# kuboyoo/alphazero-general-ori

Measured on AMD Instinct MI355X. Metric: self-play rollouts/sec (32k boards, 2p Splendor) at 1/2/4/8 MI355X, higher is better.
Workload: dtype fp32 (network) / int8 (boards) / f64 (tree statistics)

## Files before the change

alphazero-general-ori_amd/csrc/mcts.hip:

```cpp
#include <hip/hip_runtime.h>

#include <cmath>
#include <cstring>
#include <new>

#include "../../include/splendor_amd.h"

#include "board_phases.h"
#include "mcts_device.h"
#include "nn_stage.h"
#include "spl_ctx.h"

using namespace spl;

#ifndef SPL_BOUNDS_CHECK
#define SPL_BOUNDS_CHECK 0
#endif
#if SPL_BOUNDS_CHECK
__device__ unsigned long long g_bounds[4 + 64];
__device__ __noinline__ void bounds_note(int site, long long v, int t) {
    atomicAdd(&g_bounds[4 + (site & 63)], 1ull);
    if (atomicAdd(&g_bounds[0], 1ull) == 0) {
        g_bounds[1] = (unsigned long long)v; g_bounds[2] = (unsigned long long)site; g_bounds[3] = (unsigned long long)t;
    }
// ... 477 lines not shown
            const int cl = c >= 0 ? node_l(P, c) : -1;
            const bool fresh = cl >= 0 && atomicCAS(&mark[cl], 0, 1) == 0;
            const uint64_t bm = __ballot(fresh);
            if (fresh) q[tail + __popcll(bm & lanemask_lt())] = cl;
            tail += __popcll(bm);
            wave_lds_fence();
        }
    }
}

typedef uint32_t u32x4 __attribute__((ext_vector_type(4)));
struct NodeRaw {
    u32x4 q[4];
    __device__ __forceinline__ int bchild() const { return (int)q[0].x; }
    __device__ __forceinline__ bool term() const { return (q[1].y & 0xFFu) != 0; }
    __device__ __forceinline__ uint64_t ebq() const { return (uint64_t)q[2].x | ((uint64_t)q[2].y << 32); }
    __device__ __forceinline__ uint64_t vbq() const { return (uint64_t)q[2].z | ((uint64_t)q[2].w << 32); }
    __device__ __forceinline__ int ec() const { return (int)(int16_t)(q[3].x & 0xFFFFu); }
    __device__ __forceinline__ void set_runs(uint64_t e, uint64_t v) {
        q[2] = u32x4{(uint32_t)e, (uint32_t)(e >> 32), (uint32_t)v, (uint32_t)(v >> 32)};
    }
    __device__ __forceinline__ void clear_hints() { q[0].y = 0xFFFFFFFFu; q[0].z = 0xFFFFFFFFu; }
};
static_assert(sizeof(NodeRaw) == sizeof(Node) && offsetof(Node, h.bchild) == 0 && offsetof(Node, h.h2) == 4 &&
                  offsetof(Node, h.h3) == 8 && offsetof(Node, h.term) == 20 && offsetof(Node, c.ebq) == 32 &&
                  offsetof(Node, c.vbq) == 40 && offsetof(Node, c.ec) == 48,
              "NodeRaw's field offsets");

constexpr int GCT = 512, GCW8 = GCT / 64;
struct GcLds {
    int32_t wsum[GCW8];
    int32_t bc[4];
};
__device__ __forceinline__ int block_scan(int x, int &total, GcLds &L) {
    const int l = lane_id(), w = threadIdx.x >> 6;
    int incl = x;
#pragma unroll
    for (int o = 1; o < 64; o <<= 1) {
        const int y = __shfl_up(incl, o, 64);
        if (l >= o) incl += y;
    }
    if (l == 63) L.wsum[w] = incl;
    __syncthreads();
    int off = 0, tot = 0;
#pragma unroll
    for (int i = 0; i < GCW8; i++) {
// ... 842 lines not shown
        b ^= mix64(x ^ 0x13198A2E03707344ull);
    }
    k0 = a;
    k1 = b | 1ull;
}
template <int N>
__device__ __forceinline__ void lane_tree_step(int8_t *s, int a) {
    Chance ch{nullptr, 0, 0, 0, 0};
    int nxt;
    switch (move_kind_of(a)) {
        case MK_GEMS: nxt = make_move<N, MK_GEMS>(s, a, 0, true, ch); break;
        case MK_BUY: nxt = make_move<N, MK_BUY>(s, a, 0, true, ch); break;
        case MK_RESERVE: nxt = make_move<N, MK_RESERVE>(s, a, 0, true, ch); break;
        default: nxt = make_move<N, MK_BUY_RESERVED>(s, a, 0, true, ch); break;
    }
    if (nxt) lane_roll_players<N>(s, nxt);
}

#ifndef SELECT_PROBE
#define SELECT_PROBE 0
#endif
#if SELECT_PROBE
__device__ unsigned long long g_sel_probe[16];
#define SPROBE(k)                                                  \
    {                                                              \
        const uint64_t c_ = __builtin_readcyclecounter();          \
        pacc[k] += c_ - plast;                                     \
        plast = c_;                                                \
    }
#else
#define SPROBE(k)
#endif
#ifndef PATH_CHUNK
#define PATH_CHUNK 8
#endif
enum { LS_DESCEND = 0, LS_EXPAND = 1, LS_DONE = 2 };

#ifndef SELECT_ASM
#define SELECT_ASM 1
#endif
#define SEL_STORES 2
#define SEL_W_OWN 3
#define SEL_W_HINT 8
#define SEL_W_HINT1 9
static_assert(SEL_W_OWN == 1 + SEL_STORES, "own child load: behind SC + the stores");
static_assert(SEL_W_HINT == SEL_STORES + 2 * (1 + SEL_STORES) && SEL_W_HINT1 == SEL_W_HINT + 1,
              "hinted record: two levels back");
#define SEL_STR2(x) #x
#define SEL_STR(x) SEL_STR2(x)
#define SEL_BODY(SA, SC, K)                                                                     \
    "v_cmp_le_i32 vcc, 0, v240\n"                       \
    "v_cmp_le_i32 %[T], 0, v243\n"                      \
    "s_and_b64 vcc, vcc, %[T]\n"                                                               \
    "v_cmp_gt_i32 %[T], %[pcap], v233\n"                \
    "s_and_b64 vcc, vcc, %[T]\n"                                                               \
    "s_and_b64 exec, exec, vcc\n"                                                              \
    "s_cbranch_execz L_done_%=\n"                                                              \
    "v_cmp_ne_u32 vcc, v240, v234\n"                  \
    "s_and_saveexec_b64 %[SV], vcc\n"                   \
    "s_mov_b64 %[INV], exec\n"                                                                 \
    "s_cbranch_execz L_nf" K "_%=\n"                                                           \
    "v_mad_u64_u32 v[238:239], %[CC], v240, 64, %[nd]\n"                                       \
    "global_load_dwordx4 " SA ", v[238:239], off\n"                                            \
    "L_nf" K "_%=:\n"                                                                          \
    "s_mov_b64 exec, %[SV]\n"                                                                  \
    "v_cmp_gt_u32 vcc, %[lim], v242\n"                  \
    "v_cndmask_b32 v226, v240, v242, vcc\n"             \
    "v_mad_u64_u32 v[238:239], %[CC], v226, 64, %[nd]\n"                                       \
    "global_load_dwordx4 " SC ", v[238:239], off\n"                                            \
    "v_mad_u64_u32 v[238:239], %[CC], v233, 4, v[252:253]\n"         \
    "global_store_dword v[238:239], v232, off\n"                                               \
    "v_and_b32 v236, 0xffff, v243\n"                                \
    "v_bfe_u32 v237, v243, 16, 15\n"                                                           \
    "v_lshl_or_b32 v236, v237, 9, v236\n"                                                      \
    "v_mad_u64_u32 v[238:239], %[CC], v233, 4, v[254:255]\n"                                   \
    "global_store_dword v[238:239], v236, off\n"                                               \
    "v_add_u32 v233, 1, v233\n"                                                                \
    "v_mov_b32 v232, v240\n"                                                                   \
    "v_mov_b32 v234, v235\n"                       \
    "v_mov_b32 v235, v226\n"                                                                   \
    "s_cmp_eq_u64 %[INV], 0\n"                                                                 \
    "s_cbranch_scc1 L_av" K "_%=\n"                                                            \
    "s_waitcnt vmcnt(" SEL_STR(SEL_W_OWN) ")\n"          \
    "s_mov_b32 %[F], 1\n"                                                                      \
    "s_branch L_sel" K "_%=\n"                                                                 \
    "L_av" K "_%=:\n"                                   \
    "s_cmp_eq_u32 %[F], 0\n"                            \
    "s_cbranch_scc1 L_a8" K "_%=\n"                     \
    "s_waitcnt vmcnt(" SEL_STR(SEL_W_HINT1) ")\n"                                              \
    "s_branch L_a0" K "_%=\n"                                                                  \
    "L_a8" K "_%=:\n"                                                                          \
    "s_waitcnt vmcnt(" SEL_STR(SEL_W_HINT) ")\n"                                               \
    "L_a0" K "_%=:\n"                                                                          \
    "s_mov_b32 %[F], 0\n"                                                                      \
    "L_sel" K "_%=:\n"
#define SEL_TAKE(R)                                                                             \
    "v_mov_b32 v240, v" #R "\n"                                                                \
    "v_mov_b32 v241, v" #R "+1\n"
__device__ __forceinline__ void descend_linked_asm(int &node, int &depth, NodeLink &rec, const Node *nd, int pcap,
                                                   int32_t *path_n, int32_t *path_x, uint64_t runm, int lim) {
    int r0 = rec.bchild, r1 = rec.h2, r2 = rec.h3;
    int r3 = (int)((uint32_t)(uint16_t)rec.best | ((uint32_t)rec.babt << 16));
    uint64_t T, SV, INV, CC, SAVE;
    int F;
    asm volatile(
        "s_mov_b64 %[SAVE], exec\n"
        "s_mov_b32 %[F], 1\n"
        "v_mov_b32 v232, %[node]\n"
        "v_mov_b32 v233, %[depth]\n"
        "v_mov_b32 v240, %[r0]\n"
        "v_mov_b32 v241, %[r1]\n"
        "v_mov_b32 v242, %[r2]\n"
        "v_mov_b32 v243, %[r3]\n"
        "v_mov_b32 v234, -1\n"
        "v_mov_b32 v235, -1\n"
        "v_mov_b64 v[252:253], %[pn]\n"
        "v_mov_b64 v[254:255], %[pxp]\n"
        "s_and_b64 exec, exec, %[runm]\n"
        "s_cbranch_execz L_done_%=\n"
        "L_top_%=:\n"
        SEL_BODY("v[244:247]", "v[228:231]", "0")
        "v_mov_b32 v240, v244\n" "v_mov_b32 v241, v245\n" "v_mov_b32 v242, v246\n" "v_mov_b32 v243, v247\n"
        SEL_BODY("v[248:251]", "v[244:247]", "1")
        "v_mov_b32 v240, v248\n" "v_mov_b32 v241, v249\n" "v_mov_b32 v242, v250\n" "v_mov_b32 v243, v251\n"
        SEL_BODY("v[228:231]", "v[248:251]", "2")
        "v_mov_b32 v240, v228\n" "v_mov_b32 v241, v229\n" "v_mov_b32 v242, v230\n" "v_mov_b32 v243, v231\n"
        "s_branch L_top_%=\n"
        "L_done_%=:\n"
        "s_waitcnt vmcnt(0)\n"
        "s_mov_b64 exec, %[SAVE]\n"
        "v_mov_b32 %[node], v232\n"
        "v_mov_b32 %[depth], v233\n"
        "v_mov_b32 %[r0], v240\n"
        "v_mov_b32 %[r1], v241\n"
        "v_mov_b32 %[r2], v242\n"
        "v_mov_b32 %[r3], v243\n"
        : [node] "+v"(node), [depth] "+v"(depth), [r0] "+v"(r0), [r1] "+v"(r1), [r2] "+v"(r2), [r3] "+v"(r3),
          [T] "=&s"(T), [SV] "=&s"(SV), [INV] "=&s"(INV), [CC] "=&s"(CC), [SAVE] "=&s"(SAVE), [F] "=&s"(F)
        : [nd] "s"(nd), [pcap] "s"(pcap), [pn] "v"(path_n), [pxp] "v"(path_x), [runm] "s"(runm), [lim] "s"(lim)
        : "v226", "v227", "v228", "v229", "v230", "v231", "v232", "v233", "v234", "v235", "v236", "v237", "v238",
          "v239", "v240", "v241", "v242", "v243", "v244", "v245", "v246", "v247", "v248", "v249", "v250", "v251",
          "v252", "v253", "v254", "v255", "vcc", "scc", "memory");
    rec.bchild = r0; rec.h2 = r1; rec.h3 = r2;
    rec.best = (int16_t)(r3 & 0xFFFF); rec.babt = (uint16_t)((uint32_t)r3 >> 16);
}
#undef SEL_BODY
#undef SEL_TAKE

template <int N>
__global__ __launch_bounds__(64) void k_select_lanes(Pools P, SearchCfg C, int B, int lim,
                                                     int8_t *__restrict__ leaf_state,
                                                     uint8_t *__restrict__ leaf_valid) {
    using Lx = Lay<N>;
    constexpr int ST = (Lx::ROWS % 2 ? Lx::ROWS : Lx::ROWS + 1) * 8;
    __shared__ __align__(16) int8_t boards[64 * ST];
    __shared__ RunScr scr;
    const int l = lane_id();
#if SELECT_PROBE
    uint64_t pacc[6] = {0, 0, 0, 0, 0, 0}, plast = __builtin_readcyclecounter();
    const uint64_t pstart = plast;
    int plev = 0, pexp = 0;
#endif
    const int slot = blockIdx.x * 64 + l;
    const bool live = slot < B;
    const int t = live ? slot : 0;
    TreeHdr *H = P.hdr + t;
    int8_t *s = boards + l * ST;
    int sims = 0, root = -1, hdepth = 0, mv = 0, hnc = 0, hnpg = 0;
    bool act = false, noise = false, forced = false;
    if (live) {
        sims = H->sims_done;
        act = sims < H->budget && !H->overflow;
        root = H->root; hdepth = H->depth; mv = H->move_no;
        noise = H->noise_pending != 0; forced = H->forced != 0;
        hnc = H->node_count; hnpg = H->npg;
        if (!act) { leaf_valid[t] = 0; H->leaf_kind = LEAF_NONE; }
    }
    const uint64_t *nbrd = reinterpret_cast<const uint64_t *>(P.nbrd);
    const int32_t pstride = P.pcap + 1;
    int32_t *path_n = P.path_n + (size_t)t * pstride;
    int32_t *path_x = P.path_x + (size_t)t * P.pcap;
    if (act && (root < 0 || !nbrd))
        for (int u = 0; u < Conv<N>::UNITS; u++) Conv<N>::load(s, P.root_state + (size_t)t * Lx::S, u);
    const bool noised = act && root >= 0 && sims == 0 && noise;
// ... 35 lines not shown
    for (uint64_t m = __ballot(scan); m; m &= m - 1) {
        const int j = __ffsll((unsigned long long)m) - 1;
        const int nj = __builtin_amdgcn_readlane(node, j);
        NodeRun r = run_of(P.nd[nj].c);
        r.eb = (int64_t)uniform64((uint64_t)r.eb); r.vb = (int64_t)uniform64((uint64_t)r.vb);
        r.ec = uniform(r.ec);
        const Pick p = scan_run(P, r, __builtin_amdgcn_readlane(nsq.ns, j), readlane_f64(nsq.qs, j), C.cpuct, C.fpu,
                                __builtin_amdgcn_readlane((int)forced, j) != 0, __builtin_amdgcn_readlane(sims, j));
        if (l == j) { pk = p; have_pk = true; }
    }
    if (have_pk) {
        if (pk.child < 0 && pk.e == nsq.best && !noised) { pk.child = nsq.bchild; pk.cterm = nsq.bterm(); }
        else pk.cterm = pk.child >= 0 ? (int)P.nd[pk.child].h.term : 0;
    }
    int bnode = nbrd ? -1 : node;
    int miss = -1, leaf_node = -1, cbest = -1;
    uint64_t k0 = 0, k1 = 0;
    float val[4] = {0, 0, 0, 0};
    NodeLink rec = *reinterpret_cast<const NodeLink *>(&nsq);
    int tv_node = -1;
    SPROBE(0)
    while (__ballot(state != LS_DONE)) {
      while (__ballot(state == LS_DESCEND)) {
        bool run = state == LS_DESCEND && !have_pk && nbrd;
#if SELECT_ASM
        {
#if SELECT_PROBE || SPL_BOUNDS_CHECK
            const int d0 = depth;
#endif
            descend_linked_asm(node, depth, rec, P.nd, P.pcap, path_n, path_x, __ballot(run), P.npages * NPG);
#if SELECT_PROBE
            plev += depth - d0;
#endif
#if SPL_BOUNDS_CHECK
            for (int d = d0; d < depth; d++) {
                const int pn = path_n[d], c = d + 1 < depth ? path_n[d + 1] : node;
                BCHK(IN_TREE(P, t, c, H->node_count), 52, c, t, (void)0);
                BCHK(P.nd[c].h.round == P.nd[pn].h.round + 1, 30, ((long long)pn << 32) | (uint32_t)c, t, (void)0);
            }
#endif
            run = false;
        }
#endif
        while (__ballot(run)) {
            if (run) {
                const int c = rec.bchild;
                run = c >= 0 && !rec.bterm() && depth < P.pcap;
                if (run) {
                    BCHK(IN_TREE(P, t, c, H->node_count), 52, c, t, (void)0);
                    BCHK(P.nd[c].h.round == P.nd[node].h.round + 1, 30, ((long long)node << 32) | (uint32_t)c, t, (void)0);
                    const NodeLink nx = link_of(P.nd, c);
                    path_n[depth] = node; path_x[depth] = px_pack(rec.best, rec.ba());
                    depth++;
                    node = c;
                    rec = nx;
#if SELECT_PROBE
                    plev++;
#endif
                }
            }
        }
        if (state == LS_DESCEND) {
            if (depth >= P.pcap) {
                state = LS_DONE; kind = LEAF_NONE; H->overflow = 2;
            } else {
                if (!have_pk) pk = Pick{rec.best, rec.ba(), rec.bchild, rec.bterm()};
                have_pk = false;
                cbest = rec.best;
#if SELECT_PROBE
                plev++;
#endif
                path_n[depth] = node; path_x[depth] = px_pack(pk.e, pk.a);
                depth++;
                if (pk.child >= 0 && pk.cterm) {
                    kind = LEAF_TERMINAL;
                    leaf_node = pk.child;
                    tv_node = pk.child;
                    state = LS_DONE;
                } else if (pk.child >= 0 && nbrd) {
                    BCHK(IN_TREE(P, t, pk.child, H->node_count), 52, pk.child, t, (void)0);
                    rec = link_of(P.nd, pk.child);
                    node = pk.child;
                } else {
// ... 103 lines not shown
#pragma unroll
        for (int i = 0; i < 4; i++) H->leaf_v[i] = val[i];
        leaf_valid[t] = kind == LEAF_NN;
        path_n[depth] = kind == LEAF_TERMINAL ? leaf_node : -1;
    }
#if SELECT_PROBE
    SPROBE(4)
    if (l == 0) {
        for (int k = 0; k < 5; k++) atomicAdd(&g_sel_probe[k], (unsigned long long)pacc[k]);
        atomicAdd(&g_sel_probe[5], 1ull);
        atomicMax(&g_sel_probe[6], (unsigned long long)(plast - pstart));
        atomicAdd(&g_sel_probe[7], (unsigned long long)(plast - pstart));
    }
    {
        const int lmax = wave_max_i32(plev);
        int lsum = plev;
#pragma unroll
        for (int o = 32; o > 0; o >>= 1) lsum += __shfl_xor(lsum, o, 64);
        if (l == 0) {
            atomicAdd(&g_sel_probe[8], (unsigned long long)lmax);
            atomicAdd(&g_sel_probe[9], (unsigned long long)lsum);
            atomicMax(&g_sel_probe[10], (unsigned long long)lmax);
            atomicAdd(&g_sel_probe[11], (unsigned long long)pexp);
        }
    }
#endif
}

#ifndef LM_PROBE
#define LM_PROBE 0
#endif
#if LM_PROBE
constexpr int LM_PSLOTS = 4096;
__device__ unsigned long long g_lm_probe[LM_PSLOTS][8];
#define LMPROBE(k) \
    if (threadIdx.x == 0 && blockIdx.x < LM_PSLOTS) g_lm_probe[blockIdx.x][k] = __builtin_amdgcn_s_memrealtime();
#else
#define LMPROBE(k)
#endif
__device__ __forceinline__ int nonzero_bytes(uint32_t x) {
    return __popc((((x & 0x7F7F7F7Fu) + 0x7F7F7F7Fu) | x) & 0x80808080u);
}
template <int N, bool STG = false>
__global__ __launch_bounds__(256) void k_leaf_mask(Pools P, int B, int lim, const int8_t *__restrict__ leaf_state,
                                                   const uint8_t *__restrict__ leaf_valid,
                                                   uint64_t *__restrict__ leaf_mask,
// ... 971 lines not shown
        }
        if (threadIdx.x < N)
            v[(size_t)t * N + threadIdx.x] =
                (float)((threadIdx.x == 0 ? 1.0 : -1.0) *
                        (1.0 - (double)(mix64(h ^ (0xA5A5ull + threadIdx.x)) >> 40) * 0x1p-30));
        return;
    }
    for (int a = threadIdx.x; a < SPL_ACTIONS; a += 256) {
        const bool ok = (mask[(size_t)t * 7 + a / 64] >> (a % 64)) & 1;
        pi[(size_t)t * SPL_ACTIONS + a] =
            ok ? (float)((double)(1 + (mix64(h + (uint64_t)a) >> 40)) * 0x1p-24) : 0.f;
    }
    if (threadIdx.x < N)
        v[(size_t)t * N + threadIdx.x] =
            (float)((double)(mix64(h ^ (0xA5A5ull + threadIdx.x)) >> 40) * 0x1p-23 - 1.0);
}

__global__ void k_init_pools(Pools P, int B) {
    const size_t tid = (size_t)blockIdx.x * blockDim.x + threadIdx.x, nth = (size_t)gridDim.x * blockDim.x;
    const int nsh = P.npages - P.nhome * B, esh = P.epages - P.ehome * B;
    for (size_t i = tid; i < (size_t)nsh; i += nth) P.nfree[i] = (int32_t)(P.npages - 1 - i);
    for (size_t i = tid; i < (size_t)esh; i += nth) P.efree[i] = (int32_t)(P.epages - 1 - i);
    if (tid == 0) { P.alloc[0] = nsh; P.alloc[1] = esh; P.alloc[2] = 0; P.alloc[3] = 0; }
}

inline int check_launch() { return hipGetLastError() == hipSuccess ? 0 : SPL_EDEVICE; }
inline dim3 wave_grid(int B) { return dim3((unsigned)((B + WAVES - 1) / WAVES)); }

#define SPL_DISPATCH(n, CALL)                          \
    switch (n) {                                       \
        case 2: { constexpr int N = 2; CALL; break; }  \
        case 3: { constexpr int N = 3; CALL; break; }  \
        default: { constexpr int N = 4; CALL; break; } \
    }

template <class T>
T *carve(char *&p, size_t count) {
    T *r = reinterpret_cast<T *>(p);
    size_t bytes = (count * sizeof(T) + 255) & ~size_t(255);
    p += bytes;
    return r;
}

}

extern "C" {
// ... 36 lines not shown
    acc(16 * no); acc(64); acc((size_t)L.nbb * nn); acc(4 * (size_t)B); acc(4 * (size_t)B); acc(8 * no);
    L.bytes = bytes;
    return L;
}

static bool valid_cfg(const spl_ctx *ctx, int B, const spl_mcts_config *cfg) {
    if (!(ok_ctx(ctx) && B > 0 && cfg && cfg->num_sims > 0 && cfg->ratio_full > 0 &&
          cfg->node_cap > 0 && cfg->edge_cap > 0 && cfg->pool_nodes >= 0 && cfg->pool_edges >= 0))
        return false;
    const long long nmax = (long long)((cfg->node_cap + NPG - 1) / NPG) * NPG;
    const long long emax = (long long)((cfg->edge_cap + UPG - 1) / UPG) * UPG;
    const long long pn = cfg->pool_nodes > 0 ? cfg->pool_nodes : (long long)B * nmax;
    const long long pe = cfg->pool_edges > 0 ? cfg->pool_edges : (long long)B * emax;
    return cfg->node_cap <= (1 << 24) && cfg->edge_cap <= (1 << 28) && pn + NPG < (1LL << 31) &&
           pe / UPG + 1 < (1LL << 31);
}

#if SELECT_PROBE
int spl_diag_select_probe(unsigned long long *out16, int reset) {
    if (hipMemcpyFromSymbol(out16, HIP_SYMBOL(g_sel_probe), 16 * 8) != hipSuccess) return SPL_EDEVICE;
    if (reset) {
        unsigned long long z[16] = {0};
        if (hipMemcpyToSymbol(HIP_SYMBOL(g_sel_probe), z, sizeof(z)) != hipSuccess) return SPL_EDEVICE;
    }
    return 0;
}
#endif

#if GC_PROBE
int spl_diag_gc_probe(unsigned long long *out24, int reset) {
    static unsigned long long h[GC_WG_MAX_PROBE][16], hm[GC_WG_MAX_PROBE][8];
    if (hipMemcpyFromSymbol(h, HIP_SYMBOL(g_gc_probe), sizeof(h)) != hipSuccess) return SPL_EDEVICE;
    if (hipMemcpyFromSymbol(hm, HIP_SYMBOL(g_gc_probe_max), sizeof(hm)) != hipSuccess) return SPL_EDEVICE;
    for (int k = 0; k < 24; k++) out24[k] = 0;
    for (int i = 0; i < GC_WG_MAX_PROBE; i++) {
        for (int k = 0; k < 10; k++) out24[k] += h[i][k];
        if (h[i][10] > out24[10]) {
            for (int k = 10; k < 14; k++) out24[k] = h[i][k];
            for (int k = 0; k < 7; k++) out24[16 + k] = hm[i][k];
        }
    }
    if (reset) {
        memset(h, 0, sizeof(h));
        memset(hm, 0, sizeof(hm));
        if (hipMemcpyToSymbol(HIP_SYMBOL(g_gc_probe), h, sizeof(h)) != hipSuccess) return SPL_EDEVICE;
        if (hipMemcpyToSymbol(HIP_SYMBOL(g_gc_probe_max), hm, sizeof(hm)) != hipSuccess) return SPL_EDEVICE;
// ... 148 lines not shown
    const int prev = g_gc_lds_limit;
    g_gc_lds_limit = nodes < 0 ? -1 : nodes;
    return prev;
}

int spl_mcts_set_roots_active(spl_mcts *m, const int8_t *roots, const uint8_t *active, int keep_tree,
                              int force_full, void *hs) {
    if (!m || !roots) return SPL_EINVAL;
    SPL_DISPATCH(m->n, hipLaunchKernelGGL(k_set_roots<N>, wave_grid(m->B), dim3(THREADS), 0,
                                          (hipStream_t)hs, m->P, m->cfg, m->B, roots, active, keep_tree,
                                          force_full));
    launch_gc(m, (hipStream_t)hs);
    return check_launch();
}

int spl_mcts_pick_best(spl_mcts *m, const uint8_t *active, uint32_t board_base, uint32_t stream,
                       int16_t *action, void *hs) {
    if (!m || !action || stream > 0xFFFFFFu) return SPL_EINVAL;
    hipLaunchKernelGGL(k_pick_best, wave_grid(m->B), dim3(THREADS), 0, (hipStream_t)hs, m->P, m->cfg,
                       m->B, active, board_base, stream, action);
    return check_launch();
}

static int launch_select(spl_mcts *m, int8_t *leaf_state, uint64_t *leaf_mask, uint8_t *leaf_valid,
                         int32_t *leaf_index, int32_t *leaf_count, void *hs) {
    SPL_DISPATCH(m->n, hipLaunchKernelGGL(k_select_lanes<N>, dim3((unsigned)((m->B + 63) / 64)), dim3(64), 0,
                                          (hipStream_t)hs, m->P, m->cfg, m->B, mcts_lim(m),
                                          leaf_state, leaf_valid));
    char *no_stage = nullptr;
    SPL_DISPATCH(m->n, hipLaunchKernelGGL(k_leaf_mask<N>, dim3((unsigned)((m->B + 63) / 64)), dim3(256), 0,
                                          (hipStream_t)hs, m->P, m->B, mcts_lim(m), leaf_state, leaf_valid,
                                          leaf_mask, leaf_index, leaf_count, no_stage));
    return check_launch();
}

static int launch_mask_staged(int n, const Pools &P, int B, int lim, const int8_t *leaf_state,
                              const uint8_t *leaf_valid, uint64_t *leaf_mask, void *stage, void *hs) {
    int32_t *no_list = nullptr;
    char *st = static_cast<char *>(stage);
    SPL_DISPATCH(n, hipLaunchKernelGGL((k_leaf_mask<N, true>), dim3((unsigned)((B + 63) / 64)), dim3(256), 0,
                                       (hipStream_t)hs, P, B, lim, leaf_state, leaf_valid, leaf_mask, no_list,
                                       no_list, st));
    return check_launch();
}
static bool stage_args_ok(const void *leaf_state, const void *leaf_mask, const void *leaf_valid, const void *stage) {
    return leaf_state && leaf_mask && leaf_valid && stage && reinterpret_cast<uintptr_t>(leaf_state) % 4 == 0 &&
           reinterpret_cast<uintptr_t>(leaf_mask) % 8 == 0 && reinterpret_cast<uintptr_t>(leaf_valid) % 16 == 0 &&
           reinterpret_cast<uintptr_t>(stage) % 16 == 0;
}

int spl_mcts_select_staged(spl_mcts *m, int8_t *leaf_state, uint64_t *leaf_mask, uint8_t *leaf_valid, void *stage,
                           void *hs) {
    if (!m || !stage_args_ok(leaf_state, leaf_mask, leaf_valid, stage)) return SPL_EINVAL;
    SPL_DISPATCH(m->n, hipLaunchKernelGGL(k_select_lanes<N>, dim3((unsigned)((m->B + 63) / 64)), dim3(64), 0,
                                          (hipStream_t)hs, m->P, m->cfg, m->B, mcts_lim(m),
                                          leaf_state, leaf_valid));
    return launch_mask_staged(m->n, m->P, m->B, mcts_lim(m), leaf_state, leaf_valid, leaf_mask, stage, hs);
}

int spl_nn_stage_leaves(const spl_ctx *ctx, int B, const int8_t *leaf_state, const uint8_t *leaf_valid,
                        uint64_t *leaf_mask, void *stage, void *hs) {
    if (!ok_ctx(ctx) || B < 0 || !stage_args_ok(leaf_state, leaf_mask, leaf_valid, stage))
        return SPL_EINVAL;
    if (!B) return 0;
    return launch_mask_staged(ctx->n, Pools{}, B, pack_lim(ctx->token_limit, ctx->rules), leaf_state, leaf_valid,
                              leaf_mask, stage, hs);
}

int spl_mcts_select(spl_mcts *m, int8_t *leaf_state, uint64_t *leaf_mask, uint8_t *leaf_valid,
                    void *hs) {
    if (!m || !leaf_state || !leaf_mask || !leaf_valid) return SPL_EINVAL;
    return launch_select(m, leaf_state, leaf_mask, leaf_valid, nullptr, nullptr, hs);
}

int spl_mcts_select_compact(spl_mcts *m, int8_t *leaf_state, uint64_t *leaf_mask, uint8_t *leaf_valid,
                            int32_t *leaf_index, int32_t *leaf_count, void *hs) {
    if (!m || !leaf_state || !leaf_mask || !leaf_valid || !leaf_index || !leaf_count) return SPL_EINVAL;
    return launch_select(m, leaf_state, leaf_mask, leaf_valid, leaf_index, leaf_count, hs);
// ... 135 lines not shown
```

alphazero-general-ori_amd/csrc/mcts_device.h:

```cpp
#pragma once
#include "splendor_device.h"

namespace spl {

constexpr double Q_UNSET = -42.0;

struct TreeHdr {
    int32_t node_count, edge_count, root, sims_done;
    int32_t budget, full, noise_pending, depth;
    int32_t leaf_kind, player, episode_step, move_no;
    int32_t game_no, overflow, n_examples, leaf_round;
    uint64_t leaf_k0, leaf_k1;
    float leaf_v[4];
    int32_t games_done, forced, moves, wd_search;
    int32_t prunes, resets, unexpanded, gc_state;
    int64_t units_gc;
    int64_t enext;
    int32_t npg, epg, eleft, live_gc;
    int32_t root_round, gc_queued, withdrawals, gcs;
    int32_t leaf_hslot, leaf_slot;
    int32_t depth_max, depth_sum;
    int32_t resume;
    int32_t sims_backed, exact_wide, big_moves;
};
// ... 149 lines not shown
__device__ __forceinline__ int64_t unit_g(const Pools &P, int t, int v) {
    const int pi = v >> UPG_SHIFT;
    const int64_t pg = pi < P.ehome ? (int64_t)t * P.ehome + pi : (int64_t)P.etab[(size_t)t * P.eptab + pi];
    return pg * UPG + (v & (UPG - 1));
}

template <int N>
struct NodeBoard {
    static constexpr int BYTES = (Lay<N>::LS + 15) & ~15;
    static constexpr int UNITS = BYTES / 16;
};

struct SearchCfg {
    double cpuct, fpu, dir_alpha, dir_temp, prob_full;
    int num_sims, ratio_full, forced_playouts, dirichlet;
    int temp_threshold, selfplay;
    int edge_reserve;
    uint64_t seed;
    uint32_t board_base;
};

enum : uint32_t { ST_FULL = 1u << 24, ST_DIR = 2u << 24, ST_PICK = 3u << 24, ST_MOVE = 4u << 24,
                  ST_DEAL = 5u << 24, ST_BEST = 6u << 24,
                  ST_PLAYER = 8u << 24 };

__device__ __forceinline__ uint64_t wave_xor64(uint64_t x) {
#pragma unroll
    for (int o = 32; o > 0; o >>= 1) x ^= __shfl_xor(x, o, 64);
    return x;
}

__device__ __forceinline__ void wave_argmax(double &u, int &i) {
#pragma unroll
    for (int o = 32; o > 0; o >>= 1) {
        double u2 = __shfl_xor(u, o, 64);
        int i2 = __shfl_xor(i, o, 64);
        if (u2 > u || (u2 == u && i2 < i)) { u = u2; i = i2; }
    }
}

template <int CTRL>
__device__ __forceinline__ double dpp_f64(double v) {
    const int lo = __double2loint(v), hi = __double2hiint(v);
    return __hiloint2double(__builtin_amdgcn_update_dpp(hi, hi, CTRL, 0xF, 0xF, false),
                            __builtin_amdgcn_update_dpp(lo, lo, CTRL, 0xF, 0xF, false));
}
__device__ __forceinline__ double wave_max_f64(double v) {
// ... 202 lines not shown
```

alphazero-general-ori_amd/splendor/_lib.py:

```python
import ctypes as C
import os

PKG_ROOT = os.path.dirname(os.path.dirname(os.path.abspath(__file__)))
LIB_PATH = os.environ.get("SPLENDOR_AMD_LIB") or os.path.join(PKG_ROOT, "libsplendor_amd.so")

ABI_VERSION = 11
EINVAL, EDEVICE = -1, -2
ERR_BAD_ACTION, ERR_BAD_INDEX = 1, 2
BACKUP_DEFER_GC = 4
PLAYER_RANDOM, PLAYER_GREEDY, PLAYER_POLICY = 0, 1, 2
PLAYOUT_UNIFORM, PLAYOUT_BUY_FIRST = 0, 1
RULE_NO_RESERVE = 1


class NativeEngineMissing(RuntimeError):
    pass


class EngineError(RuntimeError):
    pass


_lib = None

# ... 39 lines not shown
                     C.c_uint32, _vp, _vp, _vp, _vp, _vp], C.c_int),
    "spl_playout_seq": ([C.c_void_p, C.c_int, _vp, _vp, _vp, _vp, C.c_int, C.c_int, C.c_int, C.c_uint64, _vp,
                         C.c_uint32, _vp, _vp, _vp, _vp, _vp], C.c_int),
    "spl_playout_mix": ([C.c_void_p, C.c_int, _vp, _vp, _vp, _vp, C.c_int, C.c_int, C.c_int, C.c_uint64, _vp,
                         C.c_uint32, _vp, _vp, _vp, _vp], C.c_int),
    "spl_mcts_create": ([C.c_void_p, C.c_int, C.c_void_p, C.POINTER(C.c_void_p)], C.c_int),
    "spl_mcts_destroy": ([C.c_void_p], C.c_int),
    "spl_mcts_device_bytes": ([C.c_void_p], C.c_longlong),
    "spl_mcts_plan_bytes": ([_vp, C.c_int, _vp], C.c_longlong),
    "spl_mcts_counters": ([C.c_void_p, _vp, _vp], C.c_int),
    "spl_mcts_pool_state": ([C.c_void_p, _vp, _vp], C.c_int),
    "spl_mcts_pool_pages": ([C.c_void_p, _vp], C.c_int),
    "spl_mcts_set_roots": ([C.c_void_p, _vp, C.c_int, C.c_int, _vp], C.c_int),
    "spl_mcts_set_roots_active": ([C.c_void_p, _vp, _vp, C.c_int, C.c_int, _vp], C.c_int),
    "spl_mcts_pick_best": ([C.c_void_p, _vp, C.c_uint32, C.c_uint32, _vp, _vp], C.c_int),
    "spl_mcts_select": ([C.c_void_p, _vp, _vp, _vp, _vp], C.c_int),
    "spl_mcts_select_compact": ([C.c_void_p, _vp, _vp, _vp, _vp, _vp, _vp], C.c_int),
    "spl_mcts_backup": ([C.c_void_p, _vp, _vp, _vp, _vp], C.c_int),
    "spl_mcts_backup_kind": ([C.c_void_p, _vp, _vp, _vp, C.c_int, _vp], C.c_int),
    "spl_mcts_root_stats": ([C.c_void_p, _vp, _vp, _vp, _vp, _vp, _vp], C.c_int),
    "spl_mcts_root_priors": ([C.c_void_p, _vp, _vp], C.c_int),
    "spl_mcts_headers": ([C.c_void_p, _vp, _vp], C.c_int),
    "spl_mcts_tree_sizes": ([C.c_void_p, _vp, _vp], C.c_int),
    "spl_mcts_reset_games": ([C.c_void_p, _vp], C.c_int),
    "spl_mcts_restart_games": ([C.c_void_p, _vp, _vp], C.c_int),
    "spl_mcts_commit": ([C.c_void_p, _vp], C.c_int),
    "spl_mcts_drain_examples": ([C.c_void_p, _vp, _vp, _vp, _vp, _vp, _vp, _vp, C.c_int, _vp, _vp], C.c_int),
    "spl_nn_input": ([C.c_void_p, C.c_int, _vp, _vp, _vp, _vp, _vp], C.c_int),
    "spl_hash_eval": ([C.c_void_p, C.c_int, _vp, _vp, _vp, _vp, _vp], C.c_int),
    "spl_hash_eval_mode": ([C.c_void_p, C.c_int, _vp, _vp, _vp, _vp, C.c_int, _vp], C.c_int),
}


class MctsConfig(C.Structure):
    _fields_ = [("num_sims", C.c_int), ("ratio_full", C.c_int), ("prob_full", C.c_double),
                ("cpuct", C.c_double), ("fpu", C.c_double), ("forced_playouts", C.c_int),
                ("dirichlet_alpha", C.c_double), ("dirichlet_temp", C.c_double),
                ("temp_threshold", C.c_int), ("node_cap", C.c_int), ("edge_cap", C.c_int),
                ("seed", C.c_uint64), ("board_base", C.c_uint32), ("selfplay", C.c_int),
                ("out_cap", C.c_int), ("node_boards", C.c_int), ("pool_nodes", C.c_longlong),
                ("pool_edges", C.c_longlong)]


def exported_symbols():
    return list(_SIGS)

# ... 27 lines not shown
```

include/splendor_amd.h:

```cpp
#ifndef SPLENDOR_AMD_H
#define SPLENDOR_AMD_H
#include <stdint.h>
#ifdef __cplusplus
extern "C" {
#endif

#define SPL_ABI_VERSION 11
#define SPL_ACTIONS 409
#define SPL_MASK_WORDS 7
#define SPL_EINVAL (-1)
#define SPL_EDEVICE (-2)
#define SPL_ERR_BAD_ACTION 1
#define SPL_ERR_BAD_INDEX 2

typedef struct spl_ctx spl_ctx;

int spl_abi_version(void);

int spl_ctx_create(int n_players, int token_limit, spl_ctx **out);
int spl_ctx_destroy(spl_ctx *ctx);
int spl_ctx_set_token_limit(spl_ctx *ctx, int token_limit);
#define SPL_RULE_NO_RESERVE 1
int spl_ctx_set_rules(spl_ctx *ctx, int flags);
int spl_ctx_rules(const spl_ctx *ctx);
// ... 118 lines not shown
int spl_mcts_backup(spl_mcts *m, const uint64_t *leaf_mask, const float *pi, const float *v,
                    void *hip_stream);
#define SPL_LEAF_NN 1
#define SPL_LEAF_TERMINAL 2
#define SPL_BACKUP_DEFER_GC 4
int spl_mcts_backup_kind(spl_mcts *m, const uint64_t *leaf_mask, const float *pi, const float *v, int kinds,
                         void *hip_stream);
int spl_mcts_root_priors(spl_mcts *m, float *ps, void *hip_stream);
int spl_mcts_root_stats(spl_mcts *m, int64_t *counts, double *qsa, double *probs, double *q,
                        int64_t *adjusted, void *hip_stream);
int spl_mcts_reset_games(spl_mcts *m, void *hip_stream);
int spl_mcts_restart_games(spl_mcts *m, const uint8_t *restart, void *hip_stream);
int spl_mcts_commit(spl_mcts *m, void *hip_stream);
int spl_mcts_counters(spl_mcts *m, int32_t *out, void *hip_stream);
int spl_mcts_pool_state(spl_mcts *m, int32_t *out, void *hip_stream);
int spl_mcts_pool_pages(const spl_mcts *m, long long *out4);
int spl_mcts_drain_examples(spl_mcts *m, int8_t *state, float *pi, uint64_t *valid,
                            float *winner, int32_t *scdiff, float *q, int32_t *meta, int max,
                            int32_t *n_out, void *hip_stream);
int spl_mcts_headers(spl_mcts *m, int32_t *out, void *hip_stream);

int spl_mcts_tree_sizes(spl_mcts *m, int32_t *out, void *hip_stream);

int spl_nn_input(const spl_ctx *ctx, int B, const int8_t *state, const uint64_t *mask,
                 float *x, uint8_t *valid, void *hip_stream);
int spl_hash_eval(const spl_ctx *ctx, int B, const int8_t *state, const uint64_t *mask,
                  float *pi, float *v, void *hip_stream);
int spl_hash_eval_mode(const spl_ctx *ctx, int B, const int8_t *state, const uint64_t *mask,
                       float *pi, float *v, int mode, void *hip_stream);

int spl_nn_packed_floats(int n_players);
int spl_nn_forward(int n_players, int B, const int8_t *leaf_state, const uint64_t *leaf_mask,
                   const float *packed_weights, float *pi, float *v, void *hip_stream);
int spl_nn_forward_indexed(int n_players, int B, const int8_t *leaf_state, const uint64_t *leaf_mask,
                           const int32_t *leaf_index, const int32_t *leaf_count, const float *packed_weights,
                           float *pi, float *v, void *hip_stream);
#define SPL_NN_F32 0
#define SPL_NN_BF16X2 1
#define SPL_NN_BF16 2
int spl_nn_forward_mode(int n_players, int B, const int8_t *leaf_state, const uint64_t *leaf_mask,
                        const int32_t *leaf_index, const int32_t *leaf_count,
                        const float *packed_weights, float *pi, float *v, int precision,
                        void *hip_stream);

long long spl_nn_stage_bytes(int n_players, int B);
int spl_mcts_select_staged(spl_mcts *m, int8_t *leaf_state, uint64_t *leaf_mask, uint8_t *leaf_valid,
// ... 11 lines not shown
```

Before: 77.03 million.

## Replace inline-asm select descent with C++ multi-hop hinted prefetch descent

Removes the hand-written inline-assembly descent loop and its scalar fallback. They are replaced by a C++ routine that issues loads for the best child and two hinted grandchild and great-grandchild nodes together, then advances up to three levels per iteration when the hints match. The intent is to keep the memory-latency overlap while letting the compiler schedule registers, rather than relying on hard-coded VGPRs and manual waitcnts. It also adds diagnostic entry points (hop count setting, hint scrambling, hint validity counts, probe histograms). The compiler-generated version may lose some of the precise overlap the assembly provided.

```diff
diff --git a/alphazero-general-ori_amd/csrc/mcts.hip b/alphazero-general-ori_amd/csrc/mcts.hip
--- a/alphazero-general-ori_amd/csrc/mcts.hip
+++ b/alphazero-general-ori_amd/csrc/mcts.hip
@@ -523,6 +523,17 @@
     }
     __device__ __forceinline__ void clear_hints() { q[0].y = 0xFFFFFFFFu; q[0].z = 0xFFFFFFFFu; }
 };
+__device__ __forceinline__ bool node_of_tree(const Pools &P, int t, int g, int nc) {
+    if (g < 0 || g >= P.npages * NPG) return false;
+    const int pg = g >> NPG_SHIFT;
+    if (pg < P.nhome * P.ntrees) {
+        if (pg / P.nhome != t) return false;
+    } else {
+        const int pi = P.npidx[pg];
+        if (pi < 0 || pi >= P.hdr[t].npg || P.ntab[(size_t)t * P.nptab + pi] != pg) return false;
+    }
+    return node_l(P, g) < nc;
+}
 static_assert(sizeof(NodeRaw) == sizeof(Node) && offsetof(Node, h.bchild) == 0 && offsetof(Node, h.h2) == 4 &&
                   offsetof(Node, h.h3) == 8 && offsetof(Node, h.term) == 20 && offsetof(Node, c.ebq) == 32 &&
                   offsetof(Node, c.vbq) == 40 && offsetof(Node, c.ec) == 48,
@@ -1411,7 +1422,13 @@
 #endif
 #if SELECT_PROBE
 __device__ unsigned long long g_sel_probe[16];
-#define SPROBE(k)                                                  \
+constexpr int SEL_HIST = 256;
+__device__ unsigned long long g_sel_hints[16];
+__device__ unsigned long long g_sel_hist[SEL_HIST];
+__device__ __forceinline__ int hint_class(int h, int lim, int at) {
+    return h < 0 || h >= lim ? 0 : at == -2 ? 3 : h == at ? 1 : 2;
+}
+#define SPROBE(k)                                                 \
     {                                                              \
         const uint64_t c_ = __builtin_readcyclecounter();          \
         pacc[k] += c_ - plast;                                     \
@@ -1425,119 +1442,48 @@
 #endif
 enum { LS_DESCEND = 0, LS_EXPAND = 1, LS_DONE = 2 };
 
-#ifndef SELECT_ASM
-#define SELECT_ASM 1
-#endif
-#define SEL_STORES 2
-#define SEL_W_OWN 3
-#define SEL_W_HINT 8
-#define SEL_W_HINT1 9
-static_assert(SEL_W_OWN == 1 + SEL_STORES, "own child load: behind SC + the stores");
-static_assert(SEL_W_HINT == SEL_STORES + 2 * (1 + SEL_STORES) && SEL_W_HINT1 == SEL_W_HINT + 1,
-              "hinted record: two levels back");
-#define SEL_STR2(x) #x
-#define SEL_STR(x) SEL_STR2(x)
-#define SEL_BODY(SA, SC, K)                                                                     \
-    "v_cmp_le_i32 vcc, 0, v240\n"                       \
-    "v_cmp_le_i32 %[T], 0, v243\n"                      \
-    "s_and_b64 vcc, vcc, %[T]\n"                                                               \
-    "v_cmp_gt_i32 %[T], %[pcap], v233\n"                \
-    "s_and_b64 vcc, vcc, %[T]\n"                                                               \
-    "s_and_b64 exec, exec, vcc\n"                                                              \
-    "s_cbranch_execz L_done_%=\n"                                                              \
-    "v_cmp_ne_u32 vcc, v240, v234\n"                  \
-    "s_and_saveexec_b64 %[SV], vcc\n"                   \
-    "s_mov_b64 %[INV], exec\n"                                                                 \
-    "s_cbranch_execz L_nf" K "_%=\n"                                                           \
-    "v_mad_u64_u32 v[238:239], %[CC], v240, 64, %[nd]\n"                                       \
-    "global_load_dwordx4 " SA ", v[238:239], off\n"                                            \
-    "L_nf" K "_%=:\n"                                                                          \
-    "s_mov_b64 exec, %[SV]\n"                                                                  \
-    "v_cmp_gt_u32 vcc, %[lim], v242\n"                  \
-    "v_cndmask_b32 v226, v240, v242, vcc\n"             \
-    "v_mad_u64_u32 v[238:239], %[CC], v226, 64, %[nd]\n"                                       \
-    "global_load_dwordx4 " SC ", v[238:239], off\n"                                            \
-    "v_mad_u64_u32 v[238:239], %[CC], v233, 4, v[252:253]\n"         \
-    "global_store_dword v[238:239], v232, off\n"                                               \
-    "v_and_b32 v236, 0xffff, v243\n"                                \
-    "v_bfe_u32 v237, v243, 16, 15\n"                                                           \
-    "v_lshl_or_b32 v236, v237, 9, v236\n"                                                      \
-    "v_mad_u64_u32 v[238:239], %[CC], v233, 4, v[254:255]\n"                                   \
-    "global_store_dword v[238:239], v236, off\n"                                               \
-    "v_add_u32 v233, 1, v233\n"                                                                \
-    "v_mov_b32 v232, v240\n"                                                                   \
-    "v_mov_b32 v234, v235\n"                       \
-    "v_mov_b32 v235, v226\n"                                                                   \
-    "s_cmp_eq_u64 %[INV], 0\n"                                                                 \
-    "s_cbranch_scc1 L_av" K "_%=\n"                                                            \
-    "s_waitcnt vmcnt(" SEL_STR(SEL_W_OWN) ")\n"          \
-    "s_mov_b32 %[F], 1\n"                                                                      \
-    "s_branch L_sel" K "_%=\n"                                                                 \
-    "L_av" K "_%=:\n"                                   \
-    "s_cmp_eq_u32 %[F], 0\n"                            \
-    "s_cbranch_scc1 L_a8" K "_%=\n"                     \
-    "s_waitcnt vmcnt(" SEL_STR(SEL_W_HINT1) ")\n"                                              \
-    "s_branch L_a0" K "_%=\n"                                                                  \
-    "L_a8" K "_%=:\n"                                                                          \
-    "s_waitcnt vmcnt(" SEL_STR(SEL_W_HINT) ")\n"                                               \
-    "L_a0" K "_%=:\n"                                                                          \
-    "s_mov_b32 %[F], 0\n"                                                                      \
-    "L_sel" K "_%=:\n"
-#define SEL_TAKE(R)                                                                             \
-    "v_mov_b32 v240, v" #R "\n"                                                                \
-    "v_mov_b32 v241, v" #R "+1\n"
-__device__ __forceinline__ void descend_linked_asm(int &node, int &depth, NodeLink &rec, const Node *nd, int pcap,
-                                                   int32_t *path_n, int32_t *path_x, uint64_t runm, int lim) {
-    int r0 = rec.bchild, r1 = rec.h2, r2 = rec.h3;
-    int r3 = (int)((uint32_t)(uint16_t)rec.best | ((uint32_t)rec.babt << 16));
-    uint64_t T, SV, INV, CC, SAVE;
-    int F;
-    asm volatile(
-        "s_mov_b64 %[SAVE], exec\n"
-        "s_mov_b32 %[F], 1\n"
-        "v_mov_b32 v232, %[node]\n"
-        "v_mov_b32 v233, %[depth]\n"
-        "v_mov_b32 v240, %[r0]\n"
-        "v_mov_b32 v241, %[r1]\n"
-        "v_mov_b32 v242, %[r2]\n"
-        "v_mov_b32 v243, %[r3]\n"
-        "v_mov_b32 v234, -1\n"
-        "v_mov_b32 v235, -1\n"
-        "v_mov_b64 v[252:253], %[pn]\n"
-        "v_mov_b64 v[254:255], %[pxp]\n"
-        "s_and_b64 exec, exec, %[runm]\n"
-        "s_cbranch_execz L_done_%=\n"
-        "L_top_%=:\n"
-        SEL_BODY("v[244:247]", "v[228:231]", "0")
-        "v_mov_b32 v240, v244\n" "v_mov_b32 v241, v245\n" "v_mov_b32 v242, v246\n" "v_mov_b32 v243, v247\n"
-        SEL_BODY("v[248:251]", "v[244:247]", "1")
-        "v_mov_b32 v240, v248\n" "v_mov_b32 v241, v249\n" "v_mov_b32 v242, v250\n" "v_mov_b32 v243, v251\n"
-        SEL_BODY("v[228:231]", "v[248:251]", "2")
-        "v_mov_b32 v240, v228\n" "v_mov_b32 v241, v229\n" "v_mov_b32 v242, v230\n" "v_mov_b32 v243, v231\n"
-        "s_branch L_top_%=\n"
-        "L_done_%=:\n"
-        "s_waitcnt vmcnt(0)\n"
-        "s_mov_b64 exec, %[SAVE]\n"
-        "v_mov_b32 %[node], v232\n"
-        "v_mov_b32 %[depth], v233\n"
-        "v_mov_b32 %[r0], v240\n"
-        "v_mov_b32 %[r1], v241\n"
-        "v_mov_b32 %[r2], v242\n"
-        "v_mov_b32 %[r3], v243\n"
-        : [node] "+v"(node), [depth] "+v"(depth), [r0] "+v"(r0), [r1] "+v"(r1), [r2] "+v"(r2), [r3] "+v"(r3),
-          [T] "=&s"(T), [SV] "=&s"(SV), [INV] "=&s"(INV), [CC] "=&s"(CC), [SAVE] "=&s"(SAVE), [F] "=&s"(F)
-        : [nd] "s"(nd), [pcap] "s"(pcap), [pn] "v"(path_n), [pxp] "v"(path_x), [runm] "s"(runm), [lim] "s"(lim)
-        : "v226", "v227", "v228", "v229", "v230", "v231", "v232", "v233", "v234", "v235", "v236", "v237", "v238",
-          "v239", "v240", "v241", "v242", "v243", "v244", "v245", "v246", "v247", "v248", "v249", "v250", "v251",
-          "v252", "v253", "v254", "v255", "vcc", "scc", "memory");
-    rec.bchild = r0; rec.h2 = r1; rec.h3 = r2;
-    rec.best = (int16_t)(r3 & 0xFFFF); rec.babt = (uint16_t)((uint32_t)r3 >> 16);
-}
-#undef SEL_BODY
-#undef SEL_TAKE
+__device__ __forceinline__ bool plain_link(const NodeLink &r, int depth, int pcap) {
+    return r.bchild >= 0 && !r.bterm() && depth < pcap;
+}
+__device__ __forceinline__ void descend_hops(const Pools &P, int t, bool run, int hops, int &node, int &depth,
+                                             NodeLink &rec, int32_t *path_n, int32_t *path_x) {
+    const Node *nd = P.nd;
+    const int pcap = P.pcap;
+    const uint32_t lim = (uint32_t)P.npages * NPG;
+    if (!(run && plain_link(rec, depth, pcap))) return;
+    int c1 = rec.bchild;
+    BCHK(IN_TREE(P, t, c1, P.hdr[t].node_count), 52, c1, t, c1 = node);
+    int c2 = (uint32_t)rec.h2 < lim ? rec.h2 : c1, c3 = (uint32_t)rec.h3 < lim ? rec.h3 : c1;
+    NodeLink A = link_of(nd, c1), B = link_of(nd, c2), C = link_of(nd, c3);
+    for (;;) {
+        BCHK(P.nd[c1].h.round == P.nd[node].h.round + 1, 30, ((long long)node << 32) | (uint32_t)c1, t, (void)0);
+        bool t2 = hops >= 2 && plain_link(A, depth + 1, pcap) && A.bchild == c2;
+        BCHK(!t2 || IN_TREE(P, t, c2, P.hdr[t].node_count), 52, c2, t, t2 = false);
+        BCHK(!t2 || P.nd[c2].h.round == P.nd[c1].h.round + 1, 30, ((long long)c1 << 32) | (uint32_t)c2, t, (void)0);
+        bool t3 = t2 && hops >= 3 && plain_link(B, depth + 2, pcap) && B.bchild == c3;
+        BCHK(!t3 || IN_TREE(P, t, c3, P.hdr[t].node_count), 52, c3, t, t3 = false);
+        BCHK(!t3 || P.nd[c3].h.round == P.nd[c2].h.round + 1, 30, ((long long)c2 << 32) | (uint32_t)c3, t, (void)0);
+        const int d0 = depth, n0 = node, x0 = px_pack(rec.best, rec.ba());
+        const int d1 = t2 ? d0 + 1 : d0, n1 = t2 ? c1 : n0, x1 = t2 ? px_pack(A.best, A.ba()) : x0;
+        const int d2 = t3 ? d0 + 2 : d1, n2 = t3 ? c2 : n1, x2 = t3 ? px_pack(B.best, B.ba()) : x1;
+        node = t3 ? c3 : t2 ? c2 : c1;
+        rec = t3 ? C : t2 ? B : A;
+        depth = d2 + 1;
+        const bool more = plain_link(rec, depth, pcap);
+        c1 = more ? rec.bchild : node;
+        BCHK(IN_TREE(P, t, c1, P.hdr[t].node_count), 52, c1, t, c1 = node);
+        c2 = more && (uint32_t)rec.h2 < lim ? rec.h2 : c1;
+        c3 = more && (uint32_t)rec.h3 < lim ? rec.h3 : c1;
+        A = link_of(nd, c1); B = link_of(nd, c2); C = link_of(nd, c3);
+        path_n[d0] = n0; path_x[d0] = x0;
+        path_n[d1] = n1; path_x[d1] = x1;
+        path_n[d2] = n2; path_x[d2] = x2;
+        if (!more) break;
+    }
+}
 
 template <int N>
-__global__ __launch_bounds__(64) void k_select_lanes(Pools P, SearchCfg C, int B, int lim,
+__global__ __launch_bounds__(64) void k_select_lanes(Pools P, SearchCfg C, int B, int lim, int hops,
                                                      int8_t *__restrict__ leaf_state,
                                                      uint8_t *__restrict__ leaf_valid) {
     using Lx = Lay<N>;
@@ -1549,6 +1495,7 @@
     uint64_t pacc[6] = {0, 0, 0, 0, 0, 0}, plast = __builtin_readcyclecounter();
     const uint64_t pstart = plast;
     int plev = 0, pexp = 0;
+    int phint[8] = {0, 0, 0, 0, 0, 0, 0, 0};
 #endif
     const int slot = blockIdx.x * 64 + l;
     const bool live = slot < B;
@@ -1630,43 +1577,23 @@
     SPROBE(0)
     while (__ballot(state != LS_DONE)) {
       while (__ballot(state == LS_DESCEND)) {
-        bool run = state == LS_DESCEND && !have_pk && nbrd;
-#if SELECT_ASM
         {
-#if SELECT_PROBE || SPL_BOUNDS_CHECK
+#if SELECT_PROBE
             const int d0 = depth;
 #endif
-            descend_linked_asm(node, depth, rec, P.nd, P.pcap, path_n, path_x, __ballot(run), P.npages * NPG);
+            descend_hops(P, t, state == LS_DESCEND && !have_pk && nbrd, hops, node, depth, rec, path_n, path_x);
 #if SELECT_PROBE
             plev += depth - d0;
-#endif
-#if SPL_BOUNDS_CHECK
+            SPROBE(1)
             for (int d = d0; d < depth; d++) {
-                const int pn = path_n[d], c = d + 1 < depth ? path_n[d + 1] : node;
-                BCHK(IN_TREE(P, t, c, H->node_count), 52, c, t, (void)0);
-                BCHK(P.nd[c].h.round == P.nd[pn].h.round + 1, 30, ((long long)pn << 32) | (uint32_t)c, t, (void)0);
+                const NodeLink r = link_of(P.nd, path_n[d]);
+                const int n2 = d + 2 < depth ? path_n[d + 2] : d + 2 == depth ? node : -2;
+                const int n3 = d + 3 < depth ? path_n[d + 3] : d + 3 == depth ? node : -2;
+                phint[hint_class(r.h2, P.npages * NPG, n2)]++;
+                phint[4 + hint_class(r.h3, P.npages * NPG, n3)]++;
             }
-#endif
-            run = false;
-        }
-#endif
-        while (__ballot(run)) {
-            if (run) {
-                const int c = rec.bchild;
-                run = c >= 0 && !rec.bterm() && depth < P.pcap;
-                if (run) {
-                    BCHK(IN_TREE(P, t, c, H->node_count), 52, c, t, (void)0);
-                    BCHK(P.nd[c].h.round == P.nd[node].h.round + 1, 30, ((long long)node << 32) | (uint32_t)c, t, (void)0);
-                    const NodeLink nx = link_of(P.nd, c);
-                    path_n[depth] = node; path_x[depth] = px_pack(rec.best, rec.ba());
-                    depth++;
-                    node = c;
-                    rec = nx;
-#if SELECT_PROBE
-                    plev++;
-#endif
-                }
-            }
+            SPROBE(5)
+#endif
         }
         if (state == LS_DESCEND) {
             if (depth >= P.pcap) {
@@ -1816,6 +1743,16 @@
             atomicAdd(&g_sel_probe[9], (unsigned long long)lsum);
             atomicMax(&g_sel_probe[10], (unsigned long long)lmax);
             atomicAdd(&g_sel_probe[11], (unsigned long long)pexp);
+            atomicAdd(&g_sel_hist[min(lmax, SEL_HIST - 1)], 1ull);
+        }
+        const int deepest = __ffsll((unsigned long long)__ballot(plev == lmax)) - 1;
+#pragma unroll
+        for (int k = 0; k < 8; k++) {
+            int hs = phint[k];
+#pragma unroll
+            for (int o = 32; o > 0; o >>= 1) hs += __shfl_xor(hs, o, 64);
+            if (l == 0) atomicAdd(&g_sel_hints[k], (unsigned long long)hs);
+            if (l == deepest) atomicAdd(&g_sel_hints[8 + k], (unsigned long long)phint[k]);
         }
     }
 #endif
@@ -2833,6 +2770,41 @@
     for (size_t i = tid; i < (size_t)nsh; i += nth) P.nfree[i] = (int32_t)(P.npages - 1 - i);
     for (size_t i = tid; i < (size_t)esh; i += nth) P.efree[i] = (int32_t)(P.epages - 1 - i);
     if (tid == 0) { P.alloc[0] = nsh; P.alloc[1] = esh; P.alloc[2] = 0; P.alloc[3] = 0; }
+}
+
+__global__ __launch_bounds__(256) void k_scramble_hints(Pools P, uint64_t seed) {
+    const int total = P.npages * NPG;
+    for (int g = blockIdx.x * blockDim.x + threadIdx.x; g < total; g += gridDim.x * blockDim.x) {
+        int h[2];
+#pragma unroll
+        for (int k = 0; k < 2; k++) {
+            const double u = philox_u01(seed, (uint32_t)g, ST_SCRAMBLE, (uint32_t)k);
+            const long long id = (long long)(u * 1.25 * (double)total);
+            h[k] = id < total ? (int)id : -1;
+        }
+        P.nd[g].h.h2 = h[0]; P.nd[g].h.h3 = h[1];
+    }
+}
+
+__global__ __launch_bounds__(64) void k_hint_counts(Pools P, int B, int32_t *out) {
+    const int t = blockIdx.x, l = lane_id();
+    if (t >= B) return;
+    const int nc = P.hdr[t].node_count;
+    int set = 0, own = 0, bad = 0;
+    for (int i = l; i < nc; i += 64) {
+        const NodeLink r = link_of(P.nd, node_g(P, t, i));
+        for (int k = 0; k < 2; k++) {
+            const int h = k ? r.h3 : r.h2;
+            if (h == -1) continue;
+            const bool ok = node_of_tree(P, t, h, nc);
+            set += h >= 0; own += ok; bad += !ok;
+        }
+    }
+#pragma unroll
+    for (int o = 32; o > 0; o >>= 1) {
+        set += __shfl_xor(set, o, 64); own += __shfl_xor(own, o, 64); bad += __shfl_xor(bad, o, 64);
+    }
+    if (l == 0) { out[4 * t] = nc; out[4 * t + 1] = set; out[4 * t + 2] = own; out[4 * t + 3] = bad; }
 }
 
 inline int check_launch() { return hipGetLastError() == hipSuccess ? 0 : SPL_EDEVICE; }
@@ -2915,6 +2887,16 @@
     if (reset) {
         unsigned long long z[16] = {0};
         if (hipMemcpyToSymbol(HIP_SYMBOL(g_sel_probe), z, sizeof(z)) != hipSuccess) return SPL_EDEVICE;
+    }
+    return 0;
+}
+int spl_diag_select_hints(unsigned long long *out272, int reset) {
+    if (hipMemcpyFromSymbol(out272, HIP_SYMBOL(g_sel_hints), 16 * 8) != hipSuccess) return SPL_EDEVICE;
+    if (hipMemcpyFromSymbol(out272 + 16, HIP_SYMBOL(g_sel_hist), SEL_HIST * 8) != hipSuccess) return SPL_EDEVICE;
+    if (reset) {
+        unsigned long long z[SEL_HIST] = {0};
+        if (hipMemcpyToSymbol(HIP_SYMBOL(g_sel_hints), z, 16 * 8) != hipSuccess) return SPL_EDEVICE;
+        if (hipMemcpyToSymbol(HIP_SYMBOL(g_sel_hist), z, sizeof(z)) != hipSuccess) return SPL_EDEVICE;
     }
     return 0;
 }
@@ -3109,10 +3091,32 @@
     return check_launch();
 }
 
+static int g_select_hops = 3;
+extern "C" int spl_diag_select_hops(int levels) {
+    if (levels < 1 || levels > 3) return SPL_EINVAL;
+    const int prev = g_select_hops;
+    g_select_hops = levels;
+    return prev;
+}
+
+extern "C" int spl_diag_scramble_hints(spl_mcts *m, uint64_t seed, void *hs) {
+    if (!m) return SPL_EINVAL;
+    const int total = m->P.npages * NPG;
+    if (total <= 0) return 0;
+    hipLaunchKernelGGL(k_scramble_hints, dim3((unsigned)std::min((total + 255) / 256, 2048)), dim3(256), 0,
+                       (hipStream_t)hs, m->P, seed);
+    return check_launch();
+}
+extern "C" int spl_diag_hint_counts(spl_mcts *m, int32_t *out, void *hs) {
+    if (!m || !out) return SPL_EINVAL;
+    hipLaunchKernelGGL(k_hint_counts, dim3((unsigned)m->B), dim3(64), 0, (hipStream_t)hs, m->P, m->B, out);
+    return check_launch();
+}
+
 static int launch_select(spl_mcts *m, int8_t *leaf_state, uint64_t *leaf_mask, uint8_t *leaf_valid,
                          int32_t *leaf_index, int32_t *leaf_count, void *hs) {
     SPL_DISPATCH(m->n, hipLaunchKernelGGL(k_select_lanes<N>, dim3((unsigned)((m->B + 63) / 64)), dim3(64), 0,
-                                          (hipStream_t)hs, m->P, m->cfg, m->B, mcts_lim(m),
+                                          (hipStream_t)hs, m->P, m->cfg, m->B, mcts_lim(m), g_select_hops,
                                           leaf_state, leaf_valid));
     char *no_stage = nullptr;
     SPL_DISPATCH(m->n, hipLaunchKernelGGL(k_leaf_mask<N>, dim3((unsigned)((m->B + 63) / 64)), dim3(256), 0,
@@ -3140,7 +3144,7 @@
                            void *hs) {
     if (!m || !stage_args_ok(leaf_state, leaf_mask, leaf_valid, stage)) return SPL_EINVAL;
     SPL_DISPATCH(m->n, hipLaunchKernelGGL(k_select_lanes<N>, dim3((unsigned)((m->B + 63) / 64)), dim3(64), 0,
-                                          (hipStream_t)hs, m->P, m->cfg, m->B, mcts_lim(m),
+                                          (hipStream_t)hs, m->P, m->cfg, m->B, mcts_lim(m), g_select_hops,
                                           leaf_state, leaf_valid));
     return launch_mask_staged(m->n, m->P, m->B, mcts_lim(m), leaf_state, leaf_valid, leaf_mask, stage, hs);
 }
diff --git a/alphazero-general-ori_amd/csrc/mcts_device.h b/alphazero-general-ori_amd/csrc/mcts_device.h
--- a/alphazero-general-ori_amd/csrc/mcts_device.h
+++ b/alphazero-general-ori_amd/csrc/mcts_device.h
@@ -195,7 +195,8 @@
 
 enum : uint32_t { ST_FULL = 1u << 24, ST_DIR = 2u << 24, ST_PICK = 3u << 24, ST_MOVE = 4u << 24,
                   ST_DEAL = 5u << 24, ST_BEST = 6u << 24,
-                  ST_PLAYER = 8u << 24 };
+                  ST_PLAYER = 8u << 24,
+                  ST_SCRAMBLE = 9u << 24 };
 
 __device__ __forceinline__ uint64_t wave_xor64(uint64_t x) {
 #pragma unroll
diff --git a/alphazero-general-ori_amd/splendor/_lib.py b/alphazero-general-ori_amd/splendor/_lib.py
--- a/alphazero-general-ori_amd/splendor/_lib.py
+++ b/alphazero-general-ori_amd/splendor/_lib.py
@@ -85,6 +85,9 @@
     "spl_mcts_root_priors": ([C.c_void_p, _vp, _vp], C.c_int),
     "spl_mcts_headers": ([C.c_void_p, _vp, _vp], C.c_int),
     "spl_mcts_tree_sizes": ([C.c_void_p, _vp, _vp], C.c_int),
+    "spl_diag_select_hops": ([C.c_int], C.c_int),
+    "spl_diag_scramble_hints": ([C.c_void_p, C.c_uint64, _vp], C.c_int),
+    "spl_diag_hint_counts": ([C.c_void_p, _vp, _vp], C.c_int),
     "spl_mcts_reset_games": ([C.c_void_p, _vp], C.c_int),
     "spl_mcts_restart_games": ([C.c_void_p, _vp, _vp], C.c_int),
     "spl_mcts_commit": ([C.c_void_p, _vp], C.c_int),
diff --git a/include/splendor_amd.h b/include/splendor_amd.h
--- a/include/splendor_amd.h
+++ b/include/splendor_amd.h
@@ -164,6 +164,10 @@
 
 int spl_mcts_tree_sizes(spl_mcts *m, int32_t *out, void *hip_stream);
 
+int spl_diag_select_hops(int levels);
+int spl_diag_scramble_hints(spl_mcts *m, uint64_t seed, void *hip_stream);
+int spl_diag_hint_counts(spl_mcts *m, int32_t *out, void *hip_stream);
+
 int spl_nn_input(const spl_ctx *ctx, int B, const int8_t *state, const uint64_t *mask,
                  float *x, uint8_t *valid, void *hip_stream);
 int spl_hash_eval(const spl_ctx *ctx, int B, const int8_t *state, const uint64_t *mask,
```

Result: slower. 75.91 million (-1.5%).
